# duwt/OrienMask

Measured on AMD Instinct MI355X. Metric: images/sec end-to-end (544^2, bs=32) forward+postprocess, higher is better.
Workload: dtype f32 (fp32 tensors and accumulation; products from hi/lo fp16 pairs of the fp32 operands, three fp16 MFMAs per product group)

## Files before the change

### include/orienmask_hip.h

```cpp
#ifndef ORIENMASK_HIP_H
#define ORIENMASK_HIP_H

#include <stddef.h>
#include <stdint.h>

#ifdef __cplusplus
extern "C" {
#endif

#define OM_VERSION 140

#define OM_OK 0
#define OM_EINVAL (-1)
#define OM_ESTATE (-2)
#define OM_ENOMEM (-3)
#define OM_EHIP (-4)

#define OM_MAX_SCALES 3
#define OM_MAX_ANCHORS 9

typedef struct om_model om_model;
typedef void* om_stream;

typedef struct om_layer_info {
// ... 92 lines not shown
size_t om_conv2d_winograd24_scratch_bytes(int B, int H, int W, int cin);
int om_conv2d_winograd24(const float* in, int B, int H, int W, int cin, int in_pix_stride, const float* u,
                         const float* scale, const float* shift, int cout, int leaky, const float* res,
                         int res_pix_stride, float* out, int out_pix_stride, void* scratch, size_t scratch_bytes,
                         om_stream stream);
int om_conv2d_split(const float* in, int B, int H, int W, int cin, int in_pix_stride, const void* w_split,
                    const float* scale_split, const float* shift, int cout, int ksize, int stride, int leaky, const float* res,
                    int res_pix_stride, float* out, int out_pix_stride, int out_mode, int up, int tile_bm, int tile_bn,
                    int32_t* status_dev, om_stream stream);
int om_conv2d_split_k(const float* in, int B, int H, int W, int cin, int in_pix_stride, const void* w_split,
                      const float* scale_split, const float* shift, int cout, int ksize, int stride, int leaky, const float* res,
                      int res_pix_stride, float* out, int out_pix_stride, int out_mode, int up, int tile_bm, int tile_bn,
                      int max_parts, int32_t* status_dev, om_stream stream);
int om_conv2d_split_gather(int nseg, const float* const* seg_ptr, const int* seg_channels, const int* seg_pix_stride,
                           const int* seg_up, int B, int H, int W, const void* w_split, const float* scale_split, const float* shift,
                           int cout, int leaky, float* out, int out_pix_stride, int32_t* status_dev, om_stream stream);
int om_conv2d_winograd24_split(const float* in, int B, int H, int W, int cin, int in_pix_stride, const void* u_split,
                               const float* scale_split, const float* shift, int cout, int leaky, const float* res,
                               int res_pix_stride, float* out, int out_pix_stride, void* scratch, size_t scratch_bytes,
                               int32_t* status_dev, om_stream stream);
int om_conv2d_wino14_split(const float* in, int B, int H, int W, int cin, int in_pix_stride, const void* u14_split,
                           const float* scale_split, const float* shift, int cout, int leaky, const float* res,
                           int res_pix_stride, float* out, int out_pix_stride, int32_t* status_dev, om_stream stream);
size_t om_conv2d_wino14_wide_scratch_bytes(int B, int H, int W, int cin);
int om_conv2d_wino14_wide(const float* in, int B, int H, int W, int cin, int in_pix_stride, const void* u14_split,
                          const float* scale_split, const float* shift, int cout, int leaky, const float* res,
                          int res_pix_stride, float* out, int out_pix_stride, void* scratch, size_t scratch_bytes,
                          int32_t* status_dev, om_stream stream);
int om_set_wino14_wide(int on);
int om_get_wino14_wide(void);
int om_set_stem_fusion(int which, int on);
int om_get_stem_fusion(int which);
int om_set_conv3x3_f16_variant(int mode);
int om_get_conv3x3_f16_variant(void);
int om_conv2d_stem(const float* in, int B, int H, int W, const float* w, const float* scale,
                   const float* shift, int cout, float* out, om_stream stream);
int om_conv2d_stem2_split(const float* in, int B, int H, int W, const float* w1, const float* scale1, const float* shift1,
                          const void* w2_split, const float* scale2_split, const float* shift2, int cout2, int leaky2, float* out,
                          int out_pix_stride, int32_t* status_dev, om_stream stream);
int om_conv2d_stem3_split(const float* in, int B, int H, int W, const float* w1, const float* scale1, const float* shift1,
                          const void* w2_split, const float* scale2_split, const float* shift2, int cout2, int leaky2, float* out,
                          int out_pix_stride, const void* w3_split, const float* scale3_split, const float* shift3, int cout3, int leaky3,
                          float* out3, int out3_pix_stride, int32_t* status_dev, om_stream stream);
int om_conv2d_stem2_f16(const float* in, int B, int H, int W, const float* w1, const float* scale1, const float* shift1,
                        const void* w2_f16, const float* scale2, const float* shift2, int cout2, int leaky2, void* out,
                        int out_pix_stride, om_stream stream);
// ... 213 lines not shown
```

### orienmask_amd/csrc/conv_wino14.hip

```cpp
#include "wino14_shared.h"

namespace om {

constexpr int W14_RING = 4;
constexpr int W14_EMAX = 144;
constexpr int W14_VPLANE = W14_EMAX * 4;
constexpr int W14_VBUF = 6 * W14_VPLANE;
constexpr int W14_UGRP = 3 * W14_BN * 4;
constexpr int W14_THREADS = 768;

template <int MODE>
__global__ __launch_bounds__(W14_THREADS, 3) void wino14_split_kernel(const Wino14Params p) {
    __shared__ f32x4 smem[2 * W14_VBUF + W14_RING * W14_UGRP + 1];
    int* const s_ticket = reinterpret_cast<int*>(smem + 2 * W14_VBUF + W14_RING * W14_UGRP);
    f32x4* const s_u = smem + 2 * W14_VBUF;

    const int tid = threadIdx.x;
    const int lane = tid & 63;
    const int wave = __builtin_amdgcn_readfirstlane(tid >> 6);
    const int ngroups = 6 * p.nch;

    int q_xcd = 0, q_hops = 0;
    auto draw_tile = [&]() {
        const int m_tiles = p.total_tiles / p.n_tiles;
        while (q_hops < 8) {
            const int q = (q_xcd + q_hops) & 7;
            const int pm0 = (int)((long long)m_tiles * q >> 3), pm1 = (int)((long long)m_tiles * (q + 1) >> 3);
            const int v = atomicAdd(p.ticket + q, 1);
            if (v < (pm1 - pm0) * p.n_tiles) return pm0 * p.n_tiles + v;
            ++q_hops;
        }
        return p.total_tiles;
    };
    if (tid == 512) {
        asm volatile("s_getreg_b32 %0, hwreg(HW_REG_XCC_ID)" : "=s"(q_xcd));
        q_xcd &= 7;
        s_ticket[0] = draw_tile();
    }
    asm volatile("s_waitcnt lgkmcnt(0)" ::: "memory");
    __builtin_amdgcn_s_barrier();
    int tile = __builtin_amdgcn_readfirstlane(s_ticket[0]);
    int tslot = 0;

    if (wave >= 8) {
        const int pid = tid - 512;
        const int hp2 = p.H + 2;
        const int ecount = (p.R + 2) * p.Ct;
        __builtin_amdgcn_s_setprio(3);
        const auto rs_in = __builtin_amdgcn_make_buffer_rsrc(const_cast<float*>(p.in), 0, p.in_bytes, 0x00020000);

        int xbase[3], xlds[3];
        unsigned xok[3];
        auto setup_items = [&](int tile_id) {
            Wino14Tile tl;
            wino14_decode(p, tile_id, tl);
#pragma unroll
            for (int k = 0; k < 3; ++k) {
                const int e = k < 2 ? 64 * k + (pid >> 2) : 128 + (pid >> 3);
                const int q = k < 2 ? pid & 3 : (pid >> 1) & 3;
                const int ch = k < 2 ? 4 * q : 4 * q + 2 * (pid & 1);
                const int rr = e / p.Ct, t = e - rr * p.Ct;
                const int g = tl.g0 - 1 + rr;
                const int b = g / hp2;
                const int y = g - b * hp2 - 1;
                const bool rowok = e < ecount && g >= 0 && g < p.gtot && y >= 0 && y < p.H;
                const int x0 = 4 * (tl.t0 + t) - 1;
                unsigned ok = 0;
#pragma unroll
                for (int x = 0; x < 6; ++x) ok |= (rowok && (unsigned)(x0 + x) < (unsigned)p.W ? 1u : 0u) << x;
                xok[k] = ok;
                xbase[k] = (((b * p.H + y) * p.W + x0) * p.in_ps + ch) * 4;
                const int sw = (e >> 2) & 3;
                xlds[k] = e < ecount ? e * 64 + (((q >> 1) ^ sw) * 16) + (ch & 7) * 2 : -1;
            }
        };
        f32x4 xq[2][6];
        f32x2 xp[2][6];
        auto item_offset = [&](int k, int x, int c) {
            return ((xok[k] >> x) & 1u) ? xbase[k] + x * p.in_ps * 4 + c * 64 : (int)0x80000000;
        };
        auto load_quad_px = [&](int k, int c, int x0, int x1) {
#pragma unroll
            for (int x = 0; x < 6; ++x)
                if (x >= x0 && x < x1) xq[k][x] = __builtin_bit_cast(f32x4, __builtin_amdgcn_raw_buffer_load_b128(rs_in, item_offset(k, x, c), 0, 0));
        };
        auto load_quad = [&](int k, int c) { load_quad_px(k, c, 0, 6); };
        auto load_pair_px = [&](auto buf, int c, int x0, int x1) {
// ... 115 lines not shown
            } else {
                chunk(c, I2{}, I0{});
            }
            tile = next_tile;
            tslot ^= 1;
        }
        return;
    }

    const int wm = wave >> 1, wn = wave & 1;
    const int fi = lane & 31, fk = lane >> 5;
    const int drow = lane >> 2, dcol = lane & 3;
    int dvo[2];
#pragma unroll
    for (int i = 0; i < 2; ++i) {
        const int row = 16 * (wave + 8 * i) + drow;
        dvo[i] = row * 64 + ((dcol ^ ((row >> 2) & 3)) * 16);
    }
    const auto rs_u = __builtin_amdgcn_make_buffer_rsrc(const_cast<_Float16*>(p.u), 0, p.u_bytes, 0x00020000);
    const int swB = (fi >> 2) & 3;
    const int boff_hi = (32 * wn + fi) * 4 + (fk ^ swB);
    const int boff_lo = (32 * wn + fi) * 4 + ((2 + fk) ^ swB);
    int aoff_hi[3], aoff_lo[3];
#pragma unroll
    for (int ky = 0; ky < 3; ++ky) {
        const int e = 32 * wm + fi + ky * p.Ct;
        const int sw = (e >> 2) & 3;
        aoff_hi[ky] = e * 4 + (fk ^ sw);
        aoff_lo[ky] = e * 4 + ((2 + fk) ^ sw);
    }
    auto issue_group = [&](int ubase, int g) {
        if (g < ngroups) {
            const int slot = g % W14_RING;
            const int soff = ubase + (g - g % 6 + w14_plane(g % 6)) * (W14_UGRP * 16);
            __builtin_amdgcn_raw_ptr_buffer_load_lds(rs_u, (lds_ptr_t)(s_u + slot * W14_UGRP + wave * 64), 16, dvo[0], soff, 0, 0);
            if (wave < 4)
                __builtin_amdgcn_raw_ptr_buffer_load_lds(rs_u, (lds_ptr_t)(s_u + slot * W14_UGRP + (wave + 8) * 64), 16, dvo[1], soff, 0, 0);
        }
    };
    Wino14Tile tl;
    bool first_of_wg = true;
    if (tile < p.total_tiles) {
        wino14_decode(p, tile, tl);
        const int ubase = tl.tile_n * p.nch * 6 * (W14_UGRP * 16);
        issue_group(ubase, 0);
        issue_group(ubase, 1);
        issue_group(ubase, 2);
    }
    while (tile < p.total_tiles) {
        const int ubase = tl.tile_n * p.nch * 6 * (W14_UGRP * 16);
        f32x16 acc[6];
#pragma unroll
        for (int j = 0; j < 6; ++j)
#pragma unroll
            for (int r = 0; r < 16; ++r) acc[j][r] = 0.f;
        if (W14_EPI_OPS<MODE> == 0 || first_of_wg) asm volatile("s_waitcnt vmcnt(0)" ::: "memory");
        else asm volatile("s_waitcnt vmcnt(%0)" ::"n"(W14_EPI_OPS<MODE>) : "memory");
        first_of_wg = false;
        __builtin_amdgcn_s_barrier();
        const int next_tile = __builtin_amdgcn_readfirstlane(s_ticket[tslot ^ 1]);
        f32x4 ca[4], na[4];
        auto read_a = [&](f32x4(&f)[4], const f32x4* sV, int j, int ky) {
            f[0] = sV[w14_plane(j) * W14_VPLANE + aoff_hi[ky]];
            f[1] = sV[w14_plane(j) * W14_VPLANE + aoff_lo[ky]];
        };
        auto read_b = [&](f32x4(&f)[4], int ky, int slot) {
            f[2] = s_u[slot * W14_UGRP + ky * (W14_BN * 4) + boff_hi];
            f[3] = s_u[slot * W14_UGRP + ky * (W14_BN * 4) + boff_lo];
        };
        auto read_frags = [&](f32x4(&f)[4], const f32x4* sV, int j, int ky, int slot) {
            read_a(f, sV, j, ky);
            read_b(f, ky, slot);
        };
// ... 176 lines not shown
            const int g = tl.g0 - 1 + rr;
            const int b = g / hp2;
            const int y = g - b * hp2 - 1;
            const bool ok = e < ecount && g >= 0 && g < p.gtot && y >= 0 && y < p.H && tl.t0 + t < TW;
            vsrc[i] = ok ? ((g * TW + tl.t0 + t) * 64 + ((dcol ^ sw) * 16)) : (int)0x80000000;
        }
    };
    auto issue_v_plane = [&](int c, int pl, int vb) {
        if (c >= p.nch) return;
        const int soff = (c * 6 + pl) * (p.gtot * TW * 64);
        __builtin_amdgcn_raw_ptr_buffer_load_lds(rs_v, (lds_ptr_t)(smem + vb * W14_VBUF + pl * W14_VPLANE + wave * 64), 16, vsrc[0], soff, 0, 0);
        if (wave == 0)
            __builtin_amdgcn_raw_ptr_buffer_load_lds(rs_v, (lds_ptr_t)(smem + vb * W14_VBUF + pl * W14_VPLANE + 8 * 64), 16, vsrc[1], soff, 0, 0);
    };
    f32x16 acc[2][6];
    for (;;) {
        if (tid == 0) s_ticket[0] = atomicAdd(p.ticket + 8, 1);
        __syncthreads();
        const int tile = __builtin_amdgcn_readfirstlane(s_ticket[0]);
        __syncthreads();
        if (tile >= total2) break;
        const int tn2 = tile % n_tiles2, tm = tile / n_tiles2;
        Wino14Tile tl;
        tl.g0 = (tm / p.ncb) * p.R; tl.t0 = (tm % p.ncb) * p.Ct; tl.tile_n = 2 * tn2 + (wn4 >> 1); tl.n0 = tl.tile_n * W14_BN;
        setup_v(tl);
#pragma unroll
        for (int b = 0; b < 2; ++b)
#pragma unroll
            for (int j = 0; j < 6; ++j)
#pragma unroll
                for (int r = 0; r < 16; ++r) acc[b][j][r] = 0.f;
        issue_group(tn2, 0);
#pragma unroll
        for (int pl = 0; pl < 6; ++pl) issue_v_plane(0, pl, 0);
        asm volatile("s_waitcnt vmcnt(0)" ::: "memory");
        __builtin_amdgcn_s_barrier();
        int g = 0;
        for (int c = 0; c < p.nch; ++c) {
            const f32x4* sV = smem + (c & 1) * W14_VBUF;
            auto group = [&](auto jc) {
                constexpr int j = decltype(jc)::value;
                constexpr int pl = w14_plane(j);
                const int slot = g & 1;
                issue_group(tn2, g + 1);
                issue_v_plane(c + 1, pl, (c & 1) ^ 1);
#pragma unroll
                for (int ky = 0; ky < 3; ++ky) {
// ... 46 lines not shown
        wino14_epilogue<MODE>(p, acc[1], tl, smem + W14_VBUF + wave * 256, 2 * wm2 + 1, wn4 & 1, lane, [] {});
    }
}

void wino14_geometry(int B, int H, int W, int* R, int* Ct, int* ncb, int* nrb) {
    const int TW = (W + 3) / 4;
    const long long gtot = (long long)B * (H + 2);
    double best = -1.0;
    for (int split = 1; split <= 8; ++split) {
        const int ct = (TW + split - 1) / split;
        if (ct > 64 || ct < 1) continue;
        int r = W14_BM / ct;
        while (r > 1 && (r + 2) * ct > W14_EMAX) --r;
        if (r < 1 || (r + 2) * ct > W14_EMAX) continue;
        if (r > gtot) r = (int)gtot;
        const int cbs = (TW + ct - 1) / ct;
        const long long rbs = (gtot + r - 1) / r;
        const double useful = (double)B * H * TW;
        const double util = useful / ((double)rbs * cbs * W14_BM);
        if (util > best) { best = util; *R = r; *Ct = ct; *ncb = cbs; *nrb = (int)rbs; }
    }
}

size_t wino14_weight_halfs(int cout_pad, int cin) { return (size_t)18 * cout_pad * cin * 2; }

struct Wino14Shape {
    long long npix, in_bytes, out_bytes, res_bytes, total_tiles;
    size_t u_bytes;
    int R, Ct, ncb, nrb;
    bool aligned_in;
    bool fast_io;
    bool fits() const {
        return aligned_in && in_bytes < 0x7FFFFFF0ll && npix < (1ll << 31) && R >= 1 && Ct >= 1 && total_tiles > 0 &&
               total_tiles < (1ll << 31) && u_bytes < 0x7FFFFFF0ull;
    }
};
static Wino14Shape wino14_shape(const ConvArgs& a, int in_align_bytes, int out_align_bytes, bool has_res, int res_align_bytes) {
    Wino14Shape s{};
    s.npix = (long long)a.B * a.H * a.W;
    s.in_bytes = (s.npix - 1) * a.in_pix_stride * 4 + (long long)a.cin * 4;
    s.out_bytes = ((s.npix - 1) * a.out_pix_stride + a.cout) * 4;
    s.res_bytes = has_res ? ((s.npix - 1) * a.res_pix_stride + a.cout) * 4 : 0;
    s.aligned_in = a.in_pix_stride % 4 == 0 && in_align_bytes >= 16;
    s.fast_io = a.cout % 4 == 0 && a.out_pix_stride % 4 == 0 && out_align_bytes >= 16 &&
                (!has_res || (a.res_pix_stride % 4 == 0 && res_align_bytes >= 16)) && s.out_bytes < 0x7FFFFFF0ll && s.res_bytes < 0x7FFFFFF0ll;
    wino14_geometry(a.B, a.H, a.W, &s.R, &s.Ct, &s.ncb, &s.nrb);
    s.total_tiles = (long long)s.nrb * s.ncb * (a.cout_pad / W14_BN);
    s.u_bytes = wino14_weight_halfs(a.cout_pad, a.cin) * 2;
    return s;
}
static bool wino14_layer_kind_ok(const ConvArgs& a) { return a.ks == 3 && a.stride == 1 && a.out_mode == 0 && a.cin % 16 == 0 && a.cin >= 16 && a.cout_pad % 64 == 0; }

static int wino14_fill_params(const ConvArgs& a, Wino14Params& p) {
    OM_REQUIRE(a.in && a.w && a.scale && a.shift && a.out && a.ticket, OM_EINVAL, "wino14: null pointer");
    OM_REQUIRE(wino14_layer_kind_ok(a), OM_EINVAL, "wino14: 3x3 stride-1 NHWC layers only, cin=%d cout_pad=%d", a.cin, a.cout_pad);
    OM_REQUIRE((reinterpret_cast<uintptr_t>(a.w) & 15) == 0, OM_EINVAL, "wino14: the weights must be 16-byte aligned");
    const Wino14Shape s = wino14_shape(a, align_bytes(a.in), align_bytes(a.out), a.res != nullptr, align_bytes(a.res));
    OM_REQUIRE(s.fits(), OM_EINVAL, "wino14: %d x %d x %d: input view (%lld bytes) not 16-byte aligned, or it, the weights, %lld pixels or "
               "%lld tiles (block %d x %d) out of range", a.B, a.H, a.W, s.in_bytes, s.npix, s.total_tiles, s.R, s.Ct);
    p.in = a.in; p.u = reinterpret_cast<const _Float16*>(a.w); p.scale = a.scale; p.shift = a.shift; p.res = a.res; p.out = a.out;
    p.ticket = a.ticket; p.status = a.status;
    p.B = a.B; p.H = a.H; p.W = a.W; p.in_ps = a.in_pix_stride; p.in_bytes = (int)s.in_bytes;
    p.cout = a.cout; p.out_ps = a.out_pix_stride; p.res_ps = a.res_pix_stride; p.leaky = a.leaky;
    p.fast_io = s.fast_io ? 1 : 0;
    p.out_bytes = s.fast_io ? (int)s.out_bytes : 0;
    p.res_bytes = s.fast_io ? (int)s.res_bytes : 0;
    p.R = s.R; p.Ct = s.Ct; p.ncb = s.ncb; p.gtot = a.B * (a.H + 2);
    p.n_tiles = a.cout_pad / W14_BN;
    p.nch = a.cin / 16;
    p.total_tiles = (int)s.total_tiles;
    p.u_bytes = (int)s.u_bytes;
    return OM_OK;
}

int launch_conv_wino14_split(const ConvArgs& a, hipStream_t stream) {
    Wino14Params p;
    if (int rc = wino14_fill_params(a, p)) return rc;
    const long long total = p.total_tiles;
    const long long grid = total < 256 ? total : 256;
    if (!p.fast_io) hipLaunchKernelGGL(wino14_split_kernel<2>, dim3((unsigned)grid), dim3(W14_THREADS), 0, stream, p);
    else if (a.res) hipLaunchKernelGGL(wino14_split_kernel<1>, dim3((unsigned)grid), dim3(W14_THREADS), 0, stream, p);
    else hipLaunchKernelGGL(wino14_split_kernel<0>, dim3((unsigned)grid), dim3(W14_THREADS), 0, stream, p);
    OM_CHECK_HIP(hipGetLastError());
    return OM_OK;
}

size_t wino14_wide_scratch_floats(int B, int H, int W, int cin) {
    return (size_t)(cin / 16) * 6 * B * (H + 2) * ((W + 3) / 4) * 16;
}

bool wino14_wide_supported(const ConvArgs& a, int in_align_bytes, int out_align_bytes, bool has_res, int res_align_bytes) {
    if (!wino14_layer_kind_ok(a) || a.cout_pad % 128) return false;
    const Wino14Shape s = wino14_shape(a, in_align_bytes, out_align_bytes, has_res, res_align_bytes);
    return s.fits() && s.fast_io && wino14_wide_scratch_floats(a.B, a.H, a.W, a.cin) * 4 < 0x7FFFFFF0ull;
}

int launch_conv_wino14_wide(const ConvArgs& a, float* scratch, hipStream_t stream) {
    OM_REQUIRE(scratch && (reinterpret_cast<uintptr_t>(scratch) & 15) == 0, OM_EINVAL, "wino14 wide: scratch must be 16-byte aligned");
    OM_REQUIRE(wino14_wide_supported(a, align_bytes(a.in), align_bytes(a.out), a.res != nullptr, align_bytes(a.res)), OM_EINVAL,
               "wino14 wide: cout_pad=%d must be a multiple of 128, the views 16-byte aligned and, like V, below 2 GiB", a.cout_pad);
    Wino14WideParams pw;
    if (int rc = wino14_fill_params(a, pw.k)) return rc;
    const int TW = (a.W + 3) / 4;
    pw.TW = TW;
    pw.v = reinterpret_cast<const _Float16*>(scratch);
    pw.v_bytes = (int)(wino14_wide_scratch_floats(a.B, a.H, a.W, a.cin) * 4);
    Wino14VParams pv;
    pv.in = a.in; pv.v = reinterpret_cast<_Float16*>(scratch);
    pv.B = a.B; pv.H = a.H; pv.W = a.W; pv.in_ps = a.in_pix_stride; pv.in_bytes = pw.k.in_bytes; pv.nch = pw.k.nch; pv.TW = TW; pv.gtot = pw.k.gtot;
    pv.items = (long long)a.B * a.H * TW * pv.nch * 2;
    hipLaunchKernelGGL(wino14_v_kernel, dim3((unsigned)((pv.items + 255) / 256)), dim3(256), 0, stream, pv);
    OM_CHECK_HIP(hipGetLastError());
    if (a.mid_event) OM_CHECK_HIP(hipEventRecord(a.mid_event, stream));
    const long long total2 = (long long)(pw.k.total_tiles / pw.k.n_tiles) * (pw.k.n_tiles / 2);
    const unsigned grid = (unsigned)(total2 < 256 ? total2 : 256);
    if (a.res) hipLaunchKernelGGL(wino14_wide_kernel<1>, dim3(grid), dim3(512), 0, stream, pw);
    else hipLaunchKernelGGL(wino14_wide_kernel<0>, dim3(grid), dim3(512), 0, stream, pw);
    OM_CHECK_HIP(hipGetLastError());
    return OM_OK;
}

}
```

### orienmask_amd/csrc/om_common.h

```cpp
#pragma once
#include <hip/hip_runtime.h>
#include <cstdarg>
#include <cstdint>
#include <cstdio>

#include "../../include/orienmask_hip.h"

namespace om {

void set_error(const char* fmt, ...);

#define OM_CHECK_HIP(expr)                                                              \
    do {                                                                                \
        hipError_t _e = (expr);                                                         \
        if (_e != hipSuccess) {                                                         \
            om::set_error("%s failed: %s (%s:%d)", #expr, hipGetErrorString(_e), __FILE__, __LINE__); \
            return OM_EHIP;                                                             \
        }                                                                               \
    } while (0)

#define OM_REQUIRE(cond, code, ...)                                                     \
    do {                                                                                \
        if (!(cond)) {                                                                  \
            om::set_error(__VA_ARGS__);                                                 \
// ... 83 lines not shown
size_t wino24_scratch_floats(int B, int H, int W, int C);
int launch_conv_wino14_split(const ConvArgs& a, hipStream_t stream);
size_t wino14_wide_scratch_floats(int B, int H, int W, int cin);
bool wino14_wide_supported(const ConvArgs& a, int in_align_bytes, int out_align_bytes, bool has_res, int res_align_bytes);
int launch_conv_wino14_wide(const ConvArgs& a, float* scratch, hipStream_t stream);
bool stem2_f16_supported(int B, int H, int W, int cout2, int out_pix_stride, int out_align_bytes);
int launch_conv_stem2_f16(const float* in_nchw, int B, int H, int W, const float* w1, const float* scale1, const float* shift1,
                          const void* w2_f16, const float* scale2, const float* shift2, int cout2, int leaky2, void* out_nhwc_f16,
                          int out_pix_stride, hipStream_t stream);
struct Stem2Third {
    const void* w_split;
    const float* scale_split;
    const float* shift;
    float* out;
    int cout, leaky, out_pix_stride;
};
bool stem2_split_supported(int B, int H, int W, int cout2, int out_pix_stride, int out_align_bytes, int cout3 = 0,
                           int out3_pix_stride = 0, int out3_align_bytes = 0);
int launch_conv_stem2_split(const float* in_nchw, int B, int H, int W, const float* w1, const float* scale1, const float* shift1,
                            const void* w2_split, const float* scale2_split, const float* shift2, int cout2, int leaky2,
                            float* out_nhwc, int out_pix_stride, int* status, hipStream_t stream, const Stem2Third* third = nullptr);
size_t wino14_weight_halfs(int cout_pad, int cin);
void wino14_geometry(int B, int H, int W, int* R, int* Ct, int* ncb, int* nrb);
bool wino_enabled();
int wino_bn(long long T, int cout_pad);
bool wino_fused_for(int cin);
int launch_zero_words(void* ptr, size_t n_words, hipStream_t stream);
int launch_conv_stem(const float* in_nchw, int B, int H, int W, const float* w, const float* scale,
                     const float* shift, int cout, float* out_nhwc, hipStream_t stream);

}
```

### orienmask_amd/csrc/om_model.cpp

```cpp
#include <algorithm>
#include <atomic>
#include <cstdlib>
#include <cstring>
#include <mutex>
#include <string>
#include <vector>

#include "om_common.h"

namespace om {

static thread_local char g_err[512] = "";

void set_error(const char* fmt, ...) {
    va_list ap;
    va_start(ap, fmt);
    vsnprintf(g_err, sizeof(g_err), fmt, ap);
    va_end(ap);
}

enum : int { BUF_INPUT = -1, BUF_BBOX32 = -2, BUF_BBOX16 = -3, BUF_BBOX8 = -4, BUF_ORIENS = -5 };
constexpr int HEAD_PIX_STRIDE = 256;

struct BufDef {
// ... 375 lines not shown
        }
        if (index >= 1 && index <= fused) { p.form = Form::InPrevious; return p; }
        const int Hin = H / L.in_div, Win = W / L.in_div, Ho = Hin / li.stride, Wo = Win / li.stride;
        const long long cells = (long long)B * (H / 32) * (W / 32);
        const bool on_read = (f16 || split) && !keep_all && upsample_on_read;
        if (f16) {
            p.blob = om::LayerPlan::F16; p.w_off = li.w16_off;
            p.to_side = on_read && L.side >= 0; p.gather = on_read && !L.gather.empty();
            om::ConvArgsH a{};
            layer_shape(a, L, p, B, H, W);
            if (!p.gather && om::conv3x3_f16_supported(a)) {
                om::conv3x3_tile_for_f16(B * Ho * Wo, li.cout_pad, Wo, li.cin / 32, &p.bm, &p.bn);
                p.form = p.bm == 512 ? Form::Conv3x3F16Tall : Form::Conv3x3F16;
            } else {
                om::conv_tile_for_f16(B * Ho * Wo, li.cout_pad, li.cin, &p.bm, &p.bn, p.gather);
                p.form = p.gather ? Form::IgemmF16Gather : Form::IgemmF16;
            }
            return p;
        }
        const bool latency = split && !keep_all && latency_cells > 0 && cells < latency_cells;
        p.ksplit_max = latency ? latency_ksplit : 0;
        const bool wino = li.wino_planes != 0 && om::wino_enabled();
        if (wino && split) {
            int R = 0, Ct = 0, ncb = 0, nrb = 0;
            om::wino14_geometry(B, Hin, Win, &R, &Ct, &ncb, &nrb);
            const long long tiles = (long long)nrb * ncb * (li.cout_pad / 64);
            p.blob = om::LayerPlan::SPLIT;
            if (latency && tiles <= 128) {
                p.form = Form::SplitDirect3x3;
                p.w_off = li.wsplit_direct_off; p.scale_off = li.wsplit_direct_scale_off;
                om::conv_tile_for_split(B * Hin * Win, li.cout_pad, &p.bm, &p.bn);
                return p;
            }
            p.form = Form::Wino14; p.bm = 128; p.bn = 64;
            p.w_off = li.wsplit_off; p.scale_off = li.wsplit_scale_off;
            if (switch_on(SW_W14_WIDE) && li.cin >= 512 && tiles > 256 && L.in.buf >= 0 && L.out.buf >= 0 && (!L.has_res || L.res.buf >= 0)) {
                om::ConvArgs a{};
                layer_shape(a, L, p, B, H, W);
                if (om::wino14_wide_supported(a, view_align_bytes(L.in, false), view_align_bytes(L.out, false), L.has_res,
                                              L.has_res ? view_align_bytes(L.res, false) : 0)) {
                    p.form = Form::Wino14Wide; p.bn = 128;
                    p.scratch_floats = om::wino14_wide_scratch_floats(B, Hin, Win, li.cin);
                }
            }
        } else if (wino && cells >= 1700ll) {
            p.form = Form::Wino24; p.bm = 64; p.bn = 64;
            p.w_off = li.wino_off;
            p.scratch_floats = om::wino24_scratch_floats(B, Hin, Win, li.cin);
        } else if (wino) {
            const bool fused_transform = om::wino_fused_for(li.cin);
            p.form = fused_transform ? Form::WinoFused : Form::Wino;
            p.bm = 64;
            p.bn = fused_transform ? (li.cout_pad % 128 == 0 ? 128 : 64) : om::wino_bn((long long)B * ((Hin + 1) / 2) * ((Win + 1) / 2), li.cout_pad);
            p.w_off = li.wino_alt_off;
            p.scratch_floats = om::wino_scratch_floats(B, Hin, Win, li.cin);
        } else if (split && li.wino_planes == 0) {
            p.blob = om::LayerPlan::SPLIT;
            p.w_off = li.wsplit_off; p.scale_off = li.wsplit_scale_off;
            p.to_side = on_read && L.side >= 0; p.gather = on_read && !L.gather.empty();
// ... 683 lines not shown
                                  out_pix_stride, scratch, scratch_bytes, stream, 0, nullptr);
}

int om_conv2d_winograd24_split(const float* in, int B, int H, int W, int cin, int in_pix_stride, const void* u_split,
                               const float* scale_split, const float* shift, int cout, int leaky, const float* res,
                               int res_pix_stride, float* out, int out_pix_stride, void* scratch, size_t scratch_bytes,
                               int32_t* status_dev, om_stream stream) {
    return conv2d_winograd24_impl(in, B, H, W, cin, in_pix_stride, static_cast<const float*>(u_split), scale_split, shift, cout,
                                  leaky, res, res_pix_stride, out, out_pix_stride, scratch, scratch_bytes, stream, 1, status_dev);
}

int om_conv2d_wino14_split(const float* in, int B, int H, int W, int cin, int in_pix_stride, const void* u14_split,
                           const float* scale_split, const float* shift, int cout, int leaky, const float* res,
                           int res_pix_stride, float* out, int out_pix_stride, int32_t* status_dev, om_stream stream) {
    OM_REQUIRE(B > 0 && H > 0 && W > 0, OM_EINVAL, "om_conv2d_wino14_split: bad shape");
    om::ConvArgs a;
    a.in = in; a.w = static_cast<const float*>(u14_split); a.scale = scale_split; a.shift = shift; a.res = res; a.out = out;
    om::fill_conv_shape(a, B, H, W, cin, in_pix_stride, cout, om::round_up(cout, 64), 3, 1, leaky, res_pix_stride, out_pix_stride);
    a.split = 1; a.status = status_dev;
    if (int rc = unit_ticket(static_cast<hipStream_t>(stream), &a.ticket)) return rc;
    return om::launch_conv_wino14_split(a, static_cast<hipStream_t>(stream));
}

size_t om_conv2d_wino14_wide_scratch_bytes(int B, int H, int W, int cin) {
    if (B <= 0 || H <= 0 || W <= 0 || cin <= 0 || cin % 16) return 0;
    return om::align_up(om::wino14_wide_scratch_floats(B, H, W, cin) * sizeof(float), 256);
}

int om_conv2d_wino14_wide(const float* in, int B, int H, int W, int cin, int in_pix_stride, const void* u14_split,
                          const float* scale_split, const float* shift, int cout, int leaky, const float* res,
                          int res_pix_stride, float* out, int out_pix_stride, void* scratch, size_t scratch_bytes,
                          int32_t* status_dev, om_stream stream) {
    OM_REQUIRE(B > 0 && H > 0 && W > 0, OM_EINVAL, "om_conv2d_wino14_wide: bad shape");
    OM_REQUIRE(scratch && scratch_bytes >= om_conv2d_wino14_wide_scratch_bytes(B, H, W, cin), OM_ENOMEM,
               "om_conv2d_wino14_wide: scratch too small");
    om::ConvArgs a;
    a.in = in; a.w = static_cast<const float*>(u14_split); a.scale = scale_split; a.shift = shift; a.res = res; a.out = out;
    om::fill_conv_shape(a, B, H, W, cin, in_pix_stride, cout, om::round_up(cout, 64), 3, 1, leaky, res_pix_stride, out_pix_stride);
    a.split = 1; a.status = status_dev;
    if (int rc = unit_ticket(static_cast<hipStream_t>(stream), &a.ticket)) return rc;
    return om::launch_conv_wino14_wide(a, static_cast<float*>(scratch), static_cast<hipStream_t>(stream));
}

int om_set_wino14_wide(int on) {
    OM_REQUIRE(on == 0 || on == 1, OM_EINVAL, "om_set_wino14_wide: %d", on);
    switch_flag(SW_W14_WIDE).store(on, std::memory_order_relaxed);
// ... 53 lines not shown
```

### orienmask_amd/csrc/wino14_shared.h

```cpp
#pragma once
#include <cstdlib>
#include <type_traits>

#include "conv_f16_common.h"

namespace om {

typedef _Float16 f16x4 __attribute__((ext_vector_type(4)));
typedef _Float16 f16x2 __attribute__((ext_vector_type(2)));
typedef float f32x2 __attribute__((ext_vector_type(2)));
typedef unsigned u32x2 __attribute__((ext_vector_type(2)));
typedef unsigned u32x4v __attribute__((__vector_size__(4 * sizeof(unsigned))));

constexpr int W14_BM = 128, W14_BN = 64;

struct Wino14Params {
    const float* in;
    const _Float16* u;
    const float* scale;
    const float* shift;
    const float* res;
    float* out;
    int* ticket;
    int* status;
    int B, H, W, in_ps, in_bytes;
    int cout, out_ps, res_ps, leaky, fast_io, out_bytes, res_bytes;
    int R, Ct, ncb, gtot;
    int n_tiles, total_tiles, nch;
    int u_bytes;
};

__host__ __device__ constexpr int w14_plane(int g) { return g == 0 ? 0 : g == 1 ? 5 : g - 1; }

struct Wino14Tile {
    int g0, t0, n0, tile_n;
};

__device__ __forceinline__ void wino14_decode(const Wino14Params& p, int tile, Wino14Tile& t) {
    t.tile_n = tile % p.n_tiles;
    const int tm = tile / p.n_tiles;
    const int cb = tm % p.ncb, rb = tm / p.ncb;
    t.g0 = rb * p.R; t.t0 = cb * p.Ct; t.n0 = t.tile_n * W14_BN;
}

template <int MODE> constexpr int W14_EPI_OPS = MODE == 0 ? 16 : MODE == 1 ? 28 : 0;
template <int MODE, typename F>
__device__ __forceinline__ void wino14_epilogue(const Wino14Params& p, const f32x16 (&acc)[6], const Wino14Tile& tl, f32x4* sT, int wm,
                                                int wn, int lane, F before_requests) {
    asm volatile("" : "+v"(lane));
    const int fi = lane & 31, fk = lane >> 5;
    const int hp2 = p.H + 2;
    const int c8 = lane & 7;
    const int nb = tl.n0 + 32 * wn + 4 * c8;
    const int nvalid = p.cout - nb;
    const f32x4 sc = *reinterpret_cast<const f32x4*>(p.scale + nb);
    const f32x4 sh = *reinterpret_cast<const f32x4*>(p.shift + nb);
    int pix0[4], oxe[4];
#pragma unroll
    for (int rd = 0; rd < 4; ++rd) {
        const int ml = 32 * wm + 8 * rd + (lane >> 3);
        const int r = ml / p.Ct, t = ml - r * p.Ct;
        const int gg = tl.g0 + r;
        const int b = gg / hp2;
        const int y = gg - b * hp2 - 1;
        const bool rowok = r < p.R && gg < p.gtot && y >= 0 && y < p.H && nvalid > 0;
        oxe[rd] = rowok ? 4 * (tl.t0 + t) : p.W;
        pix0[rd] = (b * p.H + y) * p.W + 4 * (tl.t0 + t);
    }
    float nonfinite = 0.f;
    auto position = [&](int px, int gq, int k) {
        const int i = 4 * gq + k;
        if (px == 0) return acc[0][i] + acc[1][i] + acc[2][i] + acc[3][i] + acc[4][i];
        if (px == 1) return (acc[1][i] - acc[2][i]) + 2.f * (acc[3][i] - acc[4][i]);
        if (px == 2) return (acc[1][i] + acc[2][i]) + 4.f * (acc[3][i] + acc[4][i]);
        return (acc[1][i] - acc[2][i]) + 8.f * (acc[3][i] - acc[4][i]) + acc[5][i];
    };
    auto transpose_in = [&](int px) {
#pragma unroll
        for (int gq = 0; gq < 4; ++gq) {
            const f32x4 v = {position(px, gq, 0), position(px, gq, 1), position(px, gq, 2), position(px, gq, 3)};
            sT[fi * 8 + ((2 * gq + fk) ^ (fi & 7))] = v;
        }
    };
    auto transpose_out = [&](int rd) {
        const int e = 8 * rd + (lane >> 3);
        return sT[e * 8 + (c8 ^ (e & 7))];
    };
    auto activate = [&](f32x4 v, bool ok) {
// ... 70 lines not shown
```

### orienmask_amd/lib.py

```python
import ctypes
import os

_HERE = os.path.dirname(os.path.abspath(__file__))
LIB_PATH = os.path.join(_HERE, "lib", "liborienmask_hip.so")

OM_MAX_SCALES = 3
OM_MAX_ANCHORS = 9
OM_STATUS_SPLIT_RANGE = 1
OM_STATUS_SK_TIMEOUT = 2


class LayerInfo(ctypes.Structure):
    _fields_ = [("name", ctypes.c_char * 64),
                ("cin", ctypes.c_int32), ("cout", ctypes.c_int32), ("cout_pad", ctypes.c_int32),
                ("ksize", ctypes.c_int32), ("stride", ctypes.c_int32),
                ("has_bn", ctypes.c_int32), ("leaky", ctypes.c_int32), ("wino_planes", ctypes.c_int32),
                ("w_off", ctypes.c_int64), ("scale_off", ctypes.c_int64), ("shift_off", ctypes.c_int64),
                ("wino_off", ctypes.c_int64), ("wino_alt_off", ctypes.c_int64), ("w16_off", ctypes.c_int64),
                ("wsplit_off", ctypes.c_int64), ("wsplit_scale_off", ctypes.c_int64),
                ("wsplit_direct_off", ctypes.c_int64), ("wsplit_direct_scale_off", ctypes.c_int64)]


class PostCfg(ctypes.Structure):
    _fields_ = [("num_scales", ctypes.c_int32),
# ... 67 lines not shown
    "om_model_create": (_i, [ctypes.POINTER(_vp), _i, _i]),
    "om_model_create_variant": (_i, [ctypes.POINTER(_vp), _i, _i, _i]),
    "om_model_destroy": (None, [_vp]),
    "om_model_num_layers": (_i, [_vp]),
    "om_model_layer_info": (_i, [_vp, _i, ctypes.POINTER(LayerInfo)]),
    "om_model_weight_floats": (_sz, [_vp]),
    "om_model_load_weights": (_i, [_vp, _vp, _sz, _i]),
    "om_model_weight_split_words": (_sz, [_vp]),
    "om_model_load_weights_split": (_i, [_vp, _vp, _sz]),
    "om_model_set_precision": (_i, [_vp, _i]),
    "om_model_get_precision": (_i, [_vp]),
    "om_model_set_latency_cells": (_i, [_vp, ctypes.c_longlong]),
    "om_model_set_latency_ksplit": (_i, [_vp, _i]),
    "om_model_attach_postprocess": (_i, [_vp, ctypes.POINTER(PostCfg), _vp, _vp, _vp, _vp, _vp, _vp, ctypes.c_size_t]),
    "om_model_set_upsample_on_read": (_i, [_vp, _i]),
    "om_conv2d_split": (_i, [_vp, _i, _i, _i, _i, _i, _vp, _vp, _vp, _i, _i, _i, _i, _vp, _i, _vp, _i, _i, _i, _i, _i, _vp, _vp]),
    "om_conv2d_split_k": (_i, [_vp, _i, _i, _i, _i, _i, _vp, _vp, _vp, _i, _i, _i, _i, _vp, _i, _vp, _i, _i, _i, _i, _i, _i, _vp, _vp]),
    "om_conv2d_winograd24_split": (_i, [_vp, _i, _i, _i, _i, _i, _vp, _vp, _vp, _i, _i, _vp, _i, _vp, _i, _vp, _sz, _vp, _vp]),
    "om_set_stem_fusion": (_i, [_i, _i]),
    "om_get_stem_fusion": (_i, [_i]),
    "om_get_conv3x3_f16_variant": (_i, []),
    "om_set_conv3x3_f16_variant": (_i, [_i]),
    "om_conv2d_wino14_split": (_i, [_vp, _i, _i, _i, _i, _i, _vp, _vp, _vp, _i, _i, _vp, _i, _vp, _i, _vp, _vp]),
    "om_conv2d_wino14_wide_scratch_bytes": (_sz, [_i, _i, _i, _i]),
    "om_conv2d_wino14_wide": (_i, [_vp, _i, _i, _i, _i, _i, _vp, _vp, _vp, _i, _i, _vp, _i, _vp, _i, _vp, _sz, _vp, _vp]),
    "om_set_wino14_wide": (_i, [_i]),
    "om_get_wino14_wide": (_i, []),
    "om_forward_workspace_bytes": (_sz, [_vp, _i, _i, _i]),
    "om_forward_status_offset": (_sz, [_vp, _i, _i, _i]),
    "om_forward": (_i, [_vp, _vp, _i, _i, _i, _vp, _vp, _vp, _vp, _vp, _sz, _vp]),
    "om_layer_tile": (_i, [_vp, _i, _i, _i, _i, ctypes.POINTER(ctypes.c_int), ctypes.POINTER(ctypes.c_int),
                           ctypes.POINTER(ctypes.c_int)]),
    "om_model_weight_halfs": (_sz, [_vp]),
    "om_model_load_weights_f16": (_i, [_vp, _vp, _sz]),
    "om_forward_f16_workspace_bytes": (_sz, [_vp, _i, _i, _i]),
    "om_forward_f16": (_i, [_vp, _vp, _i, _i, _i, _vp, _vp, _vp, _vp, _vp, _sz, _vp]),
    "om_layer_tile_f16": (_i, [_vp, _i, _i, _i, _i, ctypes.POINTER(ctypes.c_int), ctypes.POINTER(ctypes.c_int),
                               ctypes.POINTER(ctypes.c_int)]),
    "om_conv2d_f16": (_i, [_vp, _i, _i, _i, _i, _i, _vp, _vp, _vp, _i, _i, _i, _i, _vp, _i, _vp, _i, _i, _vp]),
    "om_conv2d_stem_f16": (_i, [_vp, _i, _i, _i, _vp, _vp, _vp, _i, _vp, _vp]),
    "om_conv2d_winograd_scratch_bytes": (_sz, [_i, _i, _i, _i]),
    "om_conv2d_winograd": (_i, [_vp, _i, _i, _i, _i, _i, _vp, _vp, _vp, _i, _i, _vp, _i, _vp, _i, _vp, _sz, _vp]),
    "om_layer_output_view": (_i, [_vp, _i, _i, _i, _i, _i, ctypes.POINTER(ctypes.c_size_t), ctypes.POINTER(ctypes.c_int),
                                  ctypes.POINTER(ctypes.c_int), ctypes.POINTER(ctypes.c_int)]),
    "om_model_keep_activations": (_i, [_vp, _i]),
    "om_conv2d_winograd24_scratch_bytes": (_sz, [_i, _i, _i, _i]),
# ... 112 lines not shown
```

Measured before the change: 2183.

## Tile wino14 output with two block-width classes and shared one-row image padding

Replaces the single fixed R x Ct block geometry of the fused Winograd F(4,3) kernel with a search over up to two column-block classes, each with its own width and row count. The search minimises the total number of M tiles and the wasted columns. Images are now stacked with one shared padding row (pitch H+1) instead of two. Each tile decodes its class at runtime, so the A-operand LDS offsets are recomputed per tile. The aim is to cut the padding and edge-tile waste that the fixed geometry left on 544-wide feature maps, at the cost of extra per-tile index arithmetic and a more complex decode.

```diff
diff --git a/include/orienmask_hip.h b/include/orienmask_hip.h
--- a/include/orienmask_hip.h
+++ b/include/orienmask_hip.h
@@ -138,6 +138,7 @@
 int om_conv2d_wino14_split(const float* in, int B, int H, int W, int cin, int in_pix_stride, const void* u14_split,
                            const float* scale_split, const float* shift, int cout, int leaky, const float* res,
                            int res_pix_stride, float* out, int out_pix_stride, int32_t* status_dev, om_stream stream);
+int om_conv2d_wino14_blocks(int B, int H, int W, int* classes, int* row_pitch, long long* m_tiles);
 size_t om_conv2d_wino14_wide_scratch_bytes(int B, int H, int W, int cin);
 int om_conv2d_wino14_wide(const float* in, int B, int H, int W, int cin, int in_pix_stride, const void* u14_split,
                           const float* scale_split, const float* shift, int cout, int leaky, const float* res,
diff --git a/orienmask_amd/csrc/conv_wino14.hip b/orienmask_amd/csrc/conv_wino14.hip
--- a/orienmask_amd/csrc/conv_wino14.hip
+++ b/orienmask_amd/csrc/conv_wino14.hip
@@ -44,8 +44,7 @@
 
     if (wave >= 8) {
         const int pid = tid - 512;
-        const int hp2 = p.H + 2;
-        const int ecount = (p.R + 2) * p.Ct;
+        const int hp = p.hp;
         __builtin_amdgcn_s_setprio(3);
         const auto rs_in = __builtin_amdgcn_make_buffer_rsrc(const_cast<float*>(p.in), 0, p.in_bytes, 0x00020000);
 
@@ -54,15 +53,16 @@
         auto setup_items = [&](int tile_id) {
             Wino14Tile tl;
             wino14_decode(p, tile_id, tl);
+            const int ecount = (tl.R + 2) * tl.Ct;
 #pragma unroll
             for (int k = 0; k < 3; ++k) {
                 const int e = k < 2 ? 64 * k + (pid >> 2) : 128 + (pid >> 3);
                 const int q = k < 2 ? pid & 3 : (pid >> 1) & 3;
                 const int ch = k < 2 ? 4 * q : 4 * q + 2 * (pid & 1);
-                const int rr = e / p.Ct, t = e - rr * p.Ct;
+                const int rr = e / tl.Ct, t = e - rr * tl.Ct;
                 const int g = tl.g0 - 1 + rr;
-                const int b = g / hp2;
-                const int y = g - b * hp2 - 1;
+                const int b = g / hp;
+                const int y = g - b * hp - 1;
                 const bool rowok = e < ecount && g >= 0 && g < p.gtot && y >= 0 && y < p.H;
                 const int x0 = 4 * (tl.t0 + t) - 1;
                 unsigned ok = 0;
@@ -224,13 +224,17 @@
     const int boff_hi = (32 * wn + fi) * 4 + (fk ^ swB);
     const int boff_lo = (32 * wn + fi) * 4 + ((2 + fk) ^ swB);
     int aoff_hi[3], aoff_lo[3];
-#pragma unroll
-    for (int ky = 0; ky < 3; ++ky) {
-        const int e = 32 * wm + fi + ky * p.Ct;
-        const int sw = (e >> 2) & 3;
-        aoff_hi[ky] = e * 4 + (fk ^ sw);
-        aoff_lo[ky] = e * 4 + ((2 + fk) ^ sw);
-    }
+    auto setup_aoff = [&](int Ct) {
+        int l = lane;
+        asm volatile("" : "+v"(l));
+#pragma unroll
+        for (int ky = 0; ky < 3; ++ky) {
+            const int e = 32 * wm + (l & 31) + ky * Ct;
+            const int sw = (e >> 2) & 3;
+            aoff_hi[ky] = e * 4 + ((l >> 5) ^ sw);
+            aoff_lo[ky] = e * 4 + ((2 + (l >> 5)) ^ sw);
+        }
+    };
     auto issue_group = [&](int ubase, int g) {
         if (g < ngroups) {
             const int slot = g % W14_RING;
@@ -251,6 +255,7 @@
     }
     while (tile < p.total_tiles) {
         const int ubase = tl.tile_n * p.nch * 6 * (W14_UGRP * 16);
+        setup_aoff(tl.Ct);
         f32x16 acc[6];
 #pragma unroll
         for (int j = 0; j < 6; ++j)
@@ -473,7 +478,7 @@
         if (tile >= total2) break;
         const int tn2 = tile % n_tiles2, tm = tile / n_tiles2;
         Wino14Tile tl;
-        tl.g0 = (tm / p.ncb) * p.R; tl.t0 = (tm % p.ncb) * p.Ct; tl.tile_n = 2 * tn2 + (wn4 >> 1); tl.n0 = tl.tile_n * W14_BN;
+        tl.R = p.R; tl.Ct = p.Ct; tl.g0 = (tm / p.ncb) * p.R; tl.t0 = (tm % p.ncb) * p.Ct; tl.tile_n = 2 * tn2 + (wn4 >> 1); tl.n0 = tl.tile_n * W14_BN;
         setup_v(tl);
 #pragma unroll
         for (int b = 0; b < 2; ++b)
@@ -566,20 +571,74 @@
     }
 }
 
+static int w14_rows_for(int ct, long long gtot) {
+    int r = W14_BM / ct;
+    while (r > 1 && (r + 2) * ct > W14_EMAX) --r;
+    if (r < 1 || (r + 2) * ct > W14_EMAX) return 0;
+    return r > gtot ? (int)gtot : r;
+}
+int wino14_blocks(int B, int H, int W, Wino14Class* cls, int* pitch, long long* gtot_out, long long* m_tiles) {
+    const int TW = (W + 3) / 4;
+    const long long gtot = (long long)B * (H + 1) + 1;
+    *pitch = H + 1; *gtot_out = gtot;
+    *m_tiles = 0;
+    int n = 1;
+    {
+        constexpr int CTMAX = W14_EMAX / 3;
+        const int ctmin = TW < 6 ? TW : 6, ctmax = TW < CTMAX ? TW : CTMAX;
+        long long nrb[CTMAX + 1] = {};
+        for (int ct = ctmin; ct <= ctmax; ++ct) nrb[ct] = (gtot + w14_rows_for(ct, gtot) - 1) / w14_rows_for(ct, gtot);
+        long long best[5] = {-1, 0, 0, 0, 0};
+        int ba = 0, bna = 0, bb = 0, bnb = 0;
+        auto offer = [&](int a, int na, int b, int nb) {
+            const long long key[5] = {na * nrb[a] + (nb ? nb * nrb[b] : 0), (long long)na * a + (long long)nb * b - TW, na + nb, nb ? 2 : 1, -b};
+            bool better = best[0] < 0;
+            for (int i = 0; i < 5 && !better; ++i) {
+                if (key[i] != best[i]) { better = key[i] < best[i]; break; }
+                if (i == 4) better = a > ba;
+            }
+            if (better) { for (int i = 0; i < 5; ++i) best[i] = key[i]; ba = a; bna = na; bb = b; bnb = nb; }
+        };
+        for (int a = ctmin; a <= ctmax; ++a) {
+            offer(a, (TW + a - 1) / a, 0, 0);
+            for (int b = ctmin; b < a; ++b)
+                for (int na = 1; na * a < TW && na * nrb[a] < best[0]; ++na) offer(a, na, b, (TW - na * a + b - 1) / b);
+        }
+        if (best[0] < 0) return 0;
+        for (int split = 2; split <= 8; ++split) {
+            const int ct = (TW + split - 1) / split;
+            if (ct >= ctmin || ct < 1) continue;
+            nrb[ct] = (gtot + w14_rows_for(ct, gtot) - 1) / w14_rows_for(ct, gtot);
+            const int n = (TW + ct - 1) / ct;
+            if (n * nrb[ct] < best[0]) { best[0] = n * nrb[ct]; ba = ct; bna = n; bnb = 0; }
+        }
+        cls[0] = Wino14Class{0, ba, bna, w14_rows_for(ba, gtot), (int)nrb[ba], 0};
+        if (bnb) {
+            cls[1] = Wino14Class{bna * ba, bb, bnb, w14_rows_for(bb, gtot), (int)nrb[bb], (int)(bna * nrb[ba])};
+            n = 2;
+        }
+        *m_tiles = best[0];
+    }
+    return n;
+}
+
 size_t wino14_weight_halfs(int cout_pad, int cin) { return (size_t)18 * cout_pad * cin * 2; }
 
 struct Wino14Shape {
     long long npix, in_bytes, out_bytes, res_bytes, total_tiles;
     size_t u_bytes;
     int R, Ct, ncb, nrb;
+    int ncls, hp;
+    long long gtot;
+    Wino14Class cls[W14_MAXCLS];
     bool aligned_in;
     bool fast_io;
     bool fits() const {
-        return aligned_in && in_bytes < 0x7FFFFFF0ll && npix < (1ll << 31) && R >= 1 && Ct >= 1 && total_tiles > 0 &&
+        return aligned_in && in_bytes < 0x7FFFFFF0ll && npix < (1ll << 31) && ncls >= 1 && gtot < (1ll << 31) && total_tiles > 0 &&
                total_tiles < (1ll << 31) && u_bytes < 0x7FFFFFF0ull;
     }
 };
-static Wino14Shape wino14_shape(const ConvArgs& a, int in_align_bytes, int out_align_bytes, bool has_res, int res_align_bytes) {
+static Wino14Shape wino14_shape(const ConvArgs& a, bool fused, int in_align_bytes, int out_align_bytes, bool has_res, int res_align_bytes) {
     Wino14Shape s{};
     s.npix = (long long)a.B * a.H * a.W;
     s.in_bytes = (s.npix - 1) * a.in_pix_stride * 4 + (long long)a.cin * 4;
@@ -588,20 +647,30 @@
     s.aligned_in = a.in_pix_stride % 4 == 0 && in_align_bytes >= 16;
     s.fast_io = a.cout % 4 == 0 && a.out_pix_stride % 4 == 0 && out_align_bytes >= 16 &&
                 (!has_res || (a.res_pix_stride % 4 == 0 && res_align_bytes >= 16)) && s.out_bytes < 0x7FFFFFF0ll && s.res_bytes < 0x7FFFFFF0ll;
-    wino14_geometry(a.B, a.H, a.W, &s.R, &s.Ct, &s.ncb, &s.nrb);
-    s.total_tiles = (long long)s.nrb * s.ncb * (a.cout_pad / W14_BN);
+    long long m_tiles = 0;
+    if (fused) {
+        s.ncls = wino14_blocks(a.B, a.H, a.W, s.cls, &s.hp, &s.gtot, &m_tiles);
+    } else {
+        wino14_geometry(a.B, a.H, a.W, &s.R, &s.Ct, &s.ncb, &s.nrb);
+        s.hp = a.H + 2; s.gtot = (long long)a.B * s.hp;
+        m_tiles = (long long)s.nrb * s.ncb;
+        s.ncls = s.R >= 1 && s.Ct >= 1 ? 1 : 0;
+        s.cls[0] = Wino14Class{0, s.Ct, s.ncb, s.R, s.nrb, 0};
+    }
+    if (s.ncls == 1) s.cls[1] = Wino14Class{0, s.cls[0].Ct, s.cls[0].ncb, s.cls[0].R, 0, m_tiles < (1ll << 31) ? (int)m_tiles : 0};
+    s.total_tiles = m_tiles * (a.cout_pad / W14_BN);
     s.u_bytes = wino14_weight_halfs(a.cout_pad, a.cin) * 2;
     return s;
 }
 static bool wino14_layer_kind_ok(const ConvArgs& a) { return a.ks == 3 && a.stride == 1 && a.out_mode == 0 && a.cin % 16 == 0 && a.cin >= 16 && a.cout_pad % 64 == 0; }
 
-static int wino14_fill_params(const ConvArgs& a, Wino14Params& p) {
+static int wino14_fill_params(const ConvArgs& a, bool fused, Wino14Params& p) {
     OM_REQUIRE(a.in && a.w && a.scale && a.shift && a.out && a.ticket, OM_EINVAL, "wino14: null pointer");
     OM_REQUIRE(wino14_layer_kind_ok(a), OM_EINVAL, "wino14: 3x3 stride-1 NHWC layers only, cin=%d cout_pad=%d", a.cin, a.cout_pad);
     OM_REQUIRE((reinterpret_cast<uintptr_t>(a.w) & 15) == 0, OM_EINVAL, "wino14: the weights must be 16-byte aligned");
-    const Wino14Shape s = wino14_shape(a, align_bytes(a.in), align_bytes(a.out), a.res != nullptr, align_bytes(a.res));
+    const Wino14Shape s = wino14_shape(a, fused, align_bytes(a.in), align_bytes(a.out), a.res != nullptr, align_bytes(a.res));
     OM_REQUIRE(s.fits(), OM_EINVAL, "wino14: %d x %d x %d: input view (%lld bytes) not 16-byte aligned, or it, the weights, %lld pixels or "
-               "%lld tiles (block %d x %d) out of range", a.B, a.H, a.W, s.in_bytes, s.npix, s.total_tiles, s.R, s.Ct);
+               "%lld tiles (first block %d x %d) out of range", a.B, a.H, a.W, s.in_bytes, s.npix, s.total_tiles, s.cls[0].R, s.cls[0].Ct);
     p.in = a.in; p.u = reinterpret_cast<const _Float16*>(a.w); p.scale = a.scale; p.shift = a.shift; p.res = a.res; p.out = a.out;
     p.ticket = a.ticket; p.status = a.status;
     p.B = a.B; p.H = a.H; p.W = a.W; p.in_ps = a.in_pix_stride; p.in_bytes = (int)s.in_bytes;
@@ -609,7 +678,8 @@
     p.fast_io = s.fast_io ? 1 : 0;
     p.out_bytes = s.fast_io ? (int)s.out_bytes : 0;
     p.res_bytes = s.fast_io ? (int)s.res_bytes : 0;
-    p.R = s.R; p.Ct = s.Ct; p.ncb = s.ncb; p.gtot = a.B * (a.H + 2);
+    p.R = s.R; p.Ct = s.Ct; p.ncb = s.ncb; p.gtot = (int)s.gtot; p.hp = s.hp;
+    for (int k = 0; k < W14_MAXCLS; ++k) p.cls[k] = s.cls[k];
     p.n_tiles = a.cout_pad / W14_BN;
     p.nch = a.cin / 16;
     p.total_tiles = (int)s.total_tiles;
@@ -619,7 +689,7 @@
 
 int launch_conv_wino14_split(const ConvArgs& a, hipStream_t stream) {
     Wino14Params p;
-    if (int rc = wino14_fill_params(a, p)) return rc;
+    if (int rc = wino14_fill_params(a, true, p)) return rc;
     const long long total = p.total_tiles;
     const long long grid = total < 256 ? total : 256;
     if (!p.fast_io) hipLaunchKernelGGL(wino14_split_kernel<2>, dim3((unsigned)grid), dim3(W14_THREADS), 0, stream, p);
@@ -635,7 +705,7 @@
 
 bool wino14_wide_supported(const ConvArgs& a, int in_align_bytes, int out_align_bytes, bool has_res, int res_align_bytes) {
     if (!wino14_layer_kind_ok(a) || a.cout_pad % 128) return false;
-    const Wino14Shape s = wino14_shape(a, in_align_bytes, out_align_bytes, has_res, res_align_bytes);
+    const Wino14Shape s = wino14_shape(a, false, in_align_bytes, out_align_bytes, has_res, res_align_bytes);
     return s.fits() && s.fast_io && wino14_wide_scratch_floats(a.B, a.H, a.W, a.cin) * 4 < 0x7FFFFFF0ull;
 }
 
@@ -644,7 +714,7 @@
     OM_REQUIRE(wino14_wide_supported(a, align_bytes(a.in), align_bytes(a.out), a.res != nullptr, align_bytes(a.res)), OM_EINVAL,
                "wino14 wide: cout_pad=%d must be a multiple of 128, the views 16-byte aligned and, like V, below 2 GiB", a.cout_pad);
     Wino14WideParams pw;
-    if (int rc = wino14_fill_params(a, pw.k)) return rc;
+    if (int rc = wino14_fill_params(a, false, pw.k)) return rc;
     const int TW = (a.W + 3) / 4;
     pw.TW = TW;
     pw.v = reinterpret_cast<const _Float16*>(scratch);
diff --git a/orienmask_amd/csrc/om_common.h b/orienmask_amd/csrc/om_common.h
--- a/orienmask_amd/csrc/om_common.h
+++ b/orienmask_amd/csrc/om_common.h
@@ -129,6 +129,11 @@
                             float* out_nhwc, int out_pix_stride, int* status, hipStream_t stream, const Stem2Third* third = nullptr);
 size_t wino14_weight_halfs(int cout_pad, int cin);
 void wino14_geometry(int B, int H, int W, int* R, int* Ct, int* ncb, int* nrb);
+constexpr int W14_MAXCLS = 2;
+struct Wino14Class {
+    int t0, Ct, ncb, R, nrb, m0;
+};
+int wino14_blocks(int B, int H, int W, Wino14Class* cls, int* pitch, long long* gtot, long long* m_tiles);
 bool wino_enabled();
 int wino_bn(long long T, int cout_pad);
 bool wino_fused_for(int cin);
diff --git a/orienmask_amd/csrc/om_model.cpp b/orienmask_amd/csrc/om_model.cpp
--- a/orienmask_amd/csrc/om_model.cpp
+++ b/orienmask_amd/csrc/om_model.cpp
@@ -421,9 +421,11 @@
         p.ksplit_max = latency ? latency_ksplit : 0;
         const bool wino = li.wino_planes != 0 && om::wino_enabled();
         if (wino && split) {
-            int R = 0, Ct = 0, ncb = 0, nrb = 0;
-            om::wino14_geometry(B, Hin, Win, &R, &Ct, &ncb, &nrb);
-            const long long tiles = (long long)nrb * ncb * (li.cout_pad / 64);
+            om::Wino14Class cls[om::W14_MAXCLS];
+            int pitch = 0;
+            long long gtot = 0, m_tiles = 0;
+            om::wino14_blocks(B, Hin, Win, cls, &pitch, &gtot, &m_tiles);
+            const long long tiles = m_tiles * (li.cout_pad / 64);
             p.blob = om::LayerPlan::SPLIT;
             if (latency && tiles <= 128) {
                 p.form = Form::SplitDirect3x3;
@@ -433,7 +435,9 @@
             }
             p.form = Form::Wino14; p.bm = 128; p.bn = 64;
             p.w_off = li.wsplit_off; p.scale_off = li.wsplit_scale_off;
-            if (switch_on(SW_W14_WIDE) && li.cin >= 512 && tiles > 256 && L.in.buf >= 0 && L.out.buf >= 0 && (!L.has_res || L.res.buf >= 0)) {
+            int R = 0, Ct = 0, ncb = 0, nrb = 0;
+            om::wino14_geometry(B, Hin, Win, &R, &Ct, &ncb, &nrb);
+            if (switch_on(SW_W14_WIDE) && li.cin >= 512 && (long long)nrb * ncb * (li.cout_pad / 64) > 256 && L.in.buf >= 0 && L.out.buf >= 0 && (!L.has_res || L.res.buf >= 0)) {
                 om::ConvArgs a{};
                 layer_shape(a, L, p, B, H, W);
                 if (om::wino14_wide_supported(a, view_align_bytes(L.in, false), view_align_bytes(L.out, false), L.has_res,
@@ -1163,6 +1167,18 @@
     return om::launch_conv_wino14_split(a, static_cast<hipStream_t>(stream));
 }
 
+int om_conv2d_wino14_blocks(int B, int H, int W, int* classes, int* row_pitch, long long* m_tiles) {
+    OM_REQUIRE(B > 0 && H > 0 && W > 0 && classes && row_pitch && m_tiles, OM_EINVAL, "om_conv2d_wino14_blocks: bad argument");
+    om::Wino14Class cls[om::W14_MAXCLS];
+    long long gtot = 0;
+    const int n = om::wino14_blocks(B, H, W, cls, row_pitch, &gtot, m_tiles);
+    for (int k = 0; k < n; ++k) {
+        const int v[5] = {cls[k].t0, cls[k].Ct, cls[k].ncb, cls[k].R, cls[k].nrb};
+        for (int i = 0; i < 5; ++i) classes[5 * k + i] = v[i];
+    }
+    return n;
+}
+
 size_t om_conv2d_wino14_wide_scratch_bytes(int B, int H, int W, int cin) {
     if (B <= 0 || H <= 0 || W <= 0 || cin <= 0 || cin % 16) return 0;
     return om::align_up(om::wino14_wide_scratch_floats(B, H, W, cin) * sizeof(float), 256);
diff --git a/orienmask_amd/csrc/wino14_shared.h b/orienmask_amd/csrc/wino14_shared.h
--- a/orienmask_amd/csrc/wino14_shared.h
+++ b/orienmask_amd/csrc/wino14_shared.h
@@ -25,7 +25,8 @@
     int* status;
     int B, H, W, in_ps, in_bytes;
     int cout, out_ps, res_ps, leaky, fast_io, out_bytes, res_bytes;
-    int R, Ct, ncb, gtot;
+    int R, Ct, ncb, gtot, hp;
+    Wino14Class cls[W14_MAXCLS];
     int n_tiles, total_tiles, nch;
     int u_bytes;
 };
@@ -34,13 +35,20 @@
 
 struct Wino14Tile {
     int g0, t0, n0, tile_n;
+    int R, Ct;
 };
 
 __device__ __forceinline__ void wino14_decode(const Wino14Params& p, int tile, Wino14Tile& t) {
+    static_assert(W14_MAXCLS == 2, "one comparison picks the class");
     t.tile_n = tile % p.n_tiles;
     const int tm = tile / p.n_tiles;
-    const int cb = tm % p.ncb, rb = tm / p.ncb;
-    t.g0 = rb * p.R; t.t0 = cb * p.Ct; t.n0 = t.tile_n * W14_BN;
+    const bool k = tm >= p.cls[1].m0;
+    const int ncb = k ? p.cls[1].ncb : p.cls[0].ncb;
+    const int tl = tm - (k ? p.cls[1].m0 : 0);
+    const int rb = tl / ncb, cb = tl - rb * ncb;
+    t.R = k ? p.cls[1].R : p.cls[0].R;
+    t.Ct = k ? p.cls[1].Ct : p.cls[0].Ct;
+    t.g0 = rb * t.R; t.t0 = (k ? p.cls[1].t0 : p.cls[0].t0) + cb * t.Ct; t.n0 = t.tile_n * W14_BN;
 }
 
 template <int MODE> constexpr int W14_EPI_OPS = MODE == 0 ? 16 : MODE == 1 ? 28 : 0;
@@ -49,7 +57,7 @@
                                                 int wn, int lane, F before_requests) {
     asm volatile("" : "+v"(lane));
     const int fi = lane & 31, fk = lane >> 5;
-    const int hp2 = p.H + 2;
+    const int hp = p.hp;
     const int c8 = lane & 7;
     const int nb = tl.n0 + 32 * wn + 4 * c8;
     const int nvalid = p.cout - nb;
@@ -59,11 +67,11 @@
 #pragma unroll
     for (int rd = 0; rd < 4; ++rd) {
         const int ml = 32 * wm + 8 * rd + (lane >> 3);
-        const int r = ml / p.Ct, t = ml - r * p.Ct;
+        const int r = ml / tl.Ct, t = ml - r * tl.Ct;
         const int gg = tl.g0 + r;
-        const int b = gg / hp2;
-        const int y = gg - b * hp2 - 1;
-        const bool rowok = r < p.R && gg < p.gtot && y >= 0 && y < p.H && nvalid > 0;
+        const int b = gg / hp;
+        const int y = gg - b * hp - 1;
+        const bool rowok = r < tl.R && gg < p.gtot && y >= 0 && y < p.H && nvalid > 0;
         oxe[rd] = rowok ? 4 * (tl.t0 + t) : p.W;
         pix0[rd] = (b * p.H + y) * p.W + 4 * (tl.t0 + t);
     }
diff --git a/orienmask_amd/lib.py b/orienmask_amd/lib.py
--- a/orienmask_amd/lib.py
+++ b/orienmask_amd/lib.py
@@ -113,6 +113,7 @@
     "om_get_conv3x3_f16_variant": (_i, []),
     "om_set_conv3x3_f16_variant": (_i, [_i]),
     "om_conv2d_wino14_split": (_i, [_vp, _i, _i, _i, _i, _i, _vp, _vp, _vp, _i, _i, _vp, _i, _vp, _i, _vp, _vp]),
+    "om_conv2d_wino14_blocks": (_i, [_i, _i, _i, ctypes.POINTER(_i), ctypes.POINTER(_i), ctypes.POINTER(ctypes.c_longlong)]),
     "om_conv2d_wino14_wide_scratch_bytes": (_sz, [_i, _i, _i, _i]),
     "om_conv2d_wino14_wide": (_i, [_vp, _i, _i, _i, _i, _i, _vp, _vp, _vp, _i, _i, _vp, _i, _vp, _i, _vp, _sz, _vp, _vp]),
     "om_set_wino14_wide": (_i, [_i]),
```

Result: faster. 2207, median of 6 (+1.1%).
